# tylerrleee/mcmc-gpu

Measured on AMD Instinct MI355X. Metric: chain-steps/sec on 256x256 grid x 1024 chains; accept-rate parity, higher is better.
Workload: dtype f64; 1 GPU; largeScaleChain 256x256 grid, 1024 chains/GPU, fp64, Philox spectral (Matern 0.9125) proposals, blocks 50-80, sigma_mc 5 (BASELINE configs[1]); chains_total=1024, mh_steps_per_bench_step=2048

## Files before the change

### mcmc_gpu_amd/csrc/chain_strip_kernel.hip

```cpp
#include "gsm_internal.h"
#include "device_util.h"
#include "proposal_device.h"
#include "strip_step.h"
#include <math.h>
#include <stdlib.h>
#include <algorithm>
#include <type_traits>

namespace gsm {

using namespace dev;
using strip::kST;
using strip::kSW;
using strip::kNR;

constexpr int kSUPW = 32 / kSW;
constexpr int kSMAXT = 16 / kSW;

static int strip_tile_len(const BlockTable& B) { return (B.max_bh + 2) * (B.max_bw + 2); }
static int strip_main_len(const FusedArgs& a) { return std::max(a.P.lds_main, strip_tile_len(a.T.B)); }
constexpr int kStripAux = 16 + 32 + 16 + kMathTabDoubles + 4 * kT1S + kMask1D;
size_t fused_strip_lds_doubles(const FusedArgs& a) { return (size_t)strip_main_len(a) + kStripAux; }

bool strip_table_ok(const StaticFields& S, const BlockTable& B, int lds_main, int tiles1_max, int tiles2_max) {
// ... 18 lines not shown
  double* __restrict__ mtab = red2 + 32 + 16;
  double* __restrict__ t1 = mtab + kMathTabDoubles;
  double* __restrict__ m1 = t1 + 4 * kT1S;

  const int tid = threadIdx.x;
  const int lane = tid & 63;
  const int wave = __builtin_amdgcn_readfirstlane(tid >> 6);
  const int chain = blockIdx.x;
  const int n_steps = fa.T.n_steps;
  const int gH = fa.T.S.H, gW = fa.T.S.W;
  const TS* const p_bed = (const TS*)fa.T.beds + (size_t)chain * (size_t)gH * (size_t)gW;
  const TS* const p_en = (const TS*)fa.T.energy + (size_t)chain * (size_t)gH * (size_t)gW;
  const double2* const p_st = fa.T.S.sA;
  const double two_sigma2 = fa.T.S.two_sigma2, rcp_two_sigma2 = fa.T.S.rcp_two_sigma2;
  const uint32_t n_cells = (uint32_t)gH * (uint32_t)gW;
  const crec_t rec0 = (crec_t)(uintptr_t)(fa.P.scalars + (size_t)chain * fa.P.n_steps);
  const uint64_t seed = NOISE ? 0ull : fa.P.seeds[chain];
  for (int i = tid; i < kMathTabDoubles; i += kST) mtab[i] = fa.P.mathtab[i];
  if (tid < 16) red[tid] = 0.0;
  __syncthreads();

  if (tid == 0) {
    const double h0 = fa.T.loss_sum[2 * chain], l0 = fa.T.loss_sum[2 * chain + 1];
    carry[0] = h0; carry[1] = l0; carry[2] = (h0 + l0) / two_sigma2;
  }
  __syncthreads();
  step::Window prev = {};
  const int64_t noise0 = NOISE ? (int64_t)chain * fa.P.n_steps * fa.noise_stride : 0;
  auto prop_rec = [&](crec_t r) {
    PropScalars q;
    q.scale = r->scale; q.nug = r->nug; q.aa = r->aa; q.m_const = r->m_const; q.m_kappa = r->m_kappa;
    q.bh = r->bh; q.bw = r->bw; q.fy_off = r->fy_off; q.g_off = r->g_off; q.pad = r->pad; q.mask_off = r->mask_off;
    q.m_nc = r->m_nc; q.m_m1 = r->m_m1; q.m_bh = r->m_bh; q.m_bw = r->m_bw;
    return q;
  };

  for (int s = 0; s < n_steps; ++s) {
    int ptid = tid;
    asm volatile("" : "+v"(ptid));
    auto relaunder = [&] { asm volatile("" : "+v"(ptid)); };
    const crec_t rec = rec0 + s;
    const int s_row = rec->row, s_col = rec->col, s_bh = rec->bh, s_bw = rec->bw;

    {
      const cargs_t K = kargs();
      const double* __restrict__ g1 = K->P.tab1d;
      if (tid >= kST - kMask1D) m1[tid - (kST - kMask1D)] = K->P.B.mask1d[rec->si * kMask1D + tid - (kST - kMask1D)];
      if (tid < 2 * s_bh) t1[(tid < s_bh) ? tid : kT1S + tid - s_bh] = g1[rec->t1h_off + tid];
      else if (tid >= 256 && tid < 256 + 2 * s_bw) {
        const int i = ptid - 256;
        const double v = g1[rec->t1w_off + i];
        t1[2 * kT1S + ((i < s_bw) ? i : kT1S + i - s_bw)] = (i < s_bw) ? v : -v;
      }
    }
    {
      const cargs_t K = kargs();
      const ProposeArgs pa = load_c(&K->P);
      const PropScalars q = prop_rec(rec);
      const PropGeom pg = prop_geom(pa, q.bh, q.bw);
      NoiseIn nz{nullptr, nullptr, nullptr};
      if (NOISE) {
        const cargs_t F = K;
        const int64_t o = noise0 + (int64_t)s * F->noise_stride;
        nz.re = F->noise_re + o; nz.im = F->noise_im + o;
      }
      coef_items<kST, NOISE, true>(ptid, pa, q, pg, seed, pa.step0 + s, lds, nz, mtab, pa.parseval ? red2 + 16 : nullptr);
    }
    if (step::halo_touches(step::clip_window(gH, gW, s_row, s_col, s_bh, s_bw), prev)) asm volatile("s_waitcnt vmcnt(0)" ::: "memory");
    asm volatile("s_waitcnt lgkmcnt(0)\n\ts_barrier" ::: "memory");
    const double dc0 = lds[0];
    {
      v4f64 uc[kSUPW], us[kSUPW];
      {
        const cargs_t K = kargs();
        const ProposeArgs pa = load_c(&K->P);
        const PropScalars q = prop_rec(rec);
        dft_stage1<kSW, kSUPW, kTabLds1D>(wave, ptid & 63, pa, q, prop_geom(pa, q.bh, q.bw), lds, t1, uc, us);
      }
      asm volatile("s_waitcnt lgkmcnt(0)\n\ts_barrier" ::: "memory");
      {
        const cargs_t K = kargs();
        const ProposeArgs pa = load_c(&K->P);
        relaunder();
        dft_tt_write<kSW, kSUPW>(wave, ptid & 63, prop_geom(pa, s_bh, s_bw), lds, uc, us);
      }
    }
    asm volatile("s_waitcnt lgkmcnt(0)\n\ts_barrier" ::: "memory");
    {
      const cargs_t K = kargs();
      const ProposeArgs pa = load_c(&K->P);
      const PropScalars q = prop_rec(rec);
      const PropGeom pg = prop_geom(pa, q.bh, q.bw);
      const int bw = q.bw;
      v4f64 fe[kSMAXT], fo[kSMAXT];
      const double mreg[kSMAXT][8] = {};
      relaunder();
      const int ln = ptid & 63;
      dft_stage2<kSW, kSMAXT, kTabLds1D>(wave, ln, pa, q, pg, lds, t1 + 2 * kT1S, fe, fo);
      const double gain = standardise<kSW, kSMAXT>(wave, ln, q, pg, dc0, red2, fe, fo, pa.parseval ? red2 + 16 : nullptr);
      NoiseIn nz{nullptr, nullptr, nullptr};
      if (NOISE) {
        const cargs_t F = K;
        const double* nb = F->noise_nug;
        if (nb) nz.nug = nb + noise0 + (int64_t)s * F->noise_stride;
      }
      const bool with_nugget = NOISE ? (nz.nug != nullptr) : (pa.rf.nugget_max > 0.0);
      emit_field<kSW, kSMAXT, kMaskLds1D>(wave, ln, pa, q, pg, fe, fo, mreg, gain, with_nugget, lds, [bw](int y, int x) { return (y + 1) * (bw + 2) + x + 1; }, m1);
      if (with_nugget) {
        __syncthreads();
        relaunder();
        nugget_pass<kST, NOISE>(ptid, pa, q, pg, seed, pa.step0 + s, nz, lds, [bw](int y, int x) { return (y + 1) * (bw + 2) + x + 1; }, mtab);
      }
    }
    relaunder();
    const step::Window Gw = step::clip_window(gH, gW, s_row, s_col, s_bh, s_bw);
    strip::Window G;
    {
      const cargs_t K = kargs();
      G = strip::make_window(gH, gW, s_row, s_col, s_bh, s_bw, K->T.S.tr0, K->T.S.tr1, K->T.S.tc0, K->T.S.tc1);
    }
    const strip::Cfg cfg = strip::config(G.wh, G.ww);
    const strip::Lane L = strip::lane_setup(ptid & 63, wave, cfg, G, gH, gW);
    const rsrc_t r_bed = make_rsrc(p_bed, n_cells * (uint32_t)sizeof(TS));
    const rsrc_t r_en = make_rsrc(p_en, n_cells * (uint32_t)sizeof(TS));
    const rsrc_t r_st = make_rsrc(p_st, 3u * n_cells * 16u);
    uint32_t upd_bits;
    double acc_old;
    bool guard;
    {
      double vb[kNR + 2], ve[kNR];
      double2 a2[strip::kNA];
      if (G.interior) strip::load_state<TS, true>(L, cfg.n, gW, r_bed, r_en, r_st, vb, ve, a2);
      else strip::load_state<TS, false>(L, cfg.n, gW, r_bed, r_en, r_st, vb, ve, a2);
      asm volatile("s_waitcnt lgkmcnt(0)\n\ts_barrier" ::: "memory");
      const int ts = s_bw + 2;
      auto field = [&](int jj, bool) { return lds[L.tidx + jj * ts]; };
      if (G.interior) strip::phase_a<TS, true>(L, cfg.n, gW, s_bw, r_st, field, lds, vb, ve, a2, upd_bits, acc_old, guard);
      else strip::phase_a<TS, false>(L, cfg.n, gW, s_bw, r_st, field, lds, vb, ve, a2, upd_bits, acc_old, guard);
    }
    asm volatile("s_waitcnt lgkmcnt(0)\n\ts_barrier" ::: "memory");
    double en[kNR], vn[kNR];
    {
      double acc_new;
      const cargs_t K = kargs();
      const step::StepConsts SC{K->T.S.res, K->T.S.rcp_res, K->T.S.two_res, K->T.S.rcp_two_res};
      if (G.interior) strip::phase_d<TS, FAST_DIV, true>(L, cfg.n, gW, s_bw, r_st, n_cells * 16u, SC, lds, en, acc_new);
      else strip::phase_d<TS, FAST_DIV, false>(L, cfg.n, gW, s_bw, r_st, n_cells * 16u, SC, lds, en, acc_new);
      double delta = acc_new - acc_old;
      if (guard) delta = INFINITY;
      const double w_delta = wave64_sum(delta);
      if (lane == 0) red[wave] = w_delta;
    }
    strip::read_candidate(L, cfg.n, s_bw, lds, vn);
    const double s_hi = carry[0], s_lo = carry[1];
    double loss_prev = carry[2];
    asm volatile("s_waitcnt lgkmcnt(0)\n\ts_barrier" ::: "memory");
    const double sd = strip::waves_sum(red, lane);
    double c_hi, c_lo, loss_next;
    const bool acc = step::decide<FAST_DIV>(sd, sd == INFINITY, s_hi, s_lo, two_sigma2, rcp_two_sigma2, loss_prev, rec->u, c_hi, c_lo, loss_next);
    if (acc) {
      if (G.interior) strip::commit<TS, true, false>(L, cfg.n, gW, r_bed, r_en, r_en, vn, en, upd_bits);
      else strip::commit<TS, false, false>(L, cfg.n, gW, r_bed, r_en, r_en, vn, en, upd_bits);
      loss_prev = loss_next;
      if (tid == 0) {
        double n_hi, n_lo;
        two_sum(c_hi, c_lo, n_hi, n_lo);
        carry[0] = n_hi; carry[1] = n_lo; carry[2] = loss_next;
      }
      prev = Gw;
    } else {
      prev = step::Window{};
    }
    if (tid == 0) {
      const cargs_t Ke = kargs();
      const StepArgs a = load_c(&Ke->T);
      step::write_record(a, step::record_index(a, chain, s), loss_prev, acc, s_row, s_col, s_bh, s_bw);
    }
  }
  if (tid == 0) {
    fa.T.loss_sum[2 * chain] = carry[0];
    fa.T.loss_sum[2 * chain + 1] = carry[1];
  }
}

template <typename TS, bool FAST_DIV>
__global__ __launch_bounds__(kST, 4) void step_strip_kernel(const StepArgs a) {
  extern __shared__ double tile[];
  __shared__ double red[16];
  __shared__ int tab[2 * 64];
  const StaticFields& S = a.S;
  const int tid = threadIdx.x;
  const int lane = tid & 63;
  const int wave = __builtin_amdgcn_readfirstlane(tid >> 6);
  const int chain = blockIdx.x;
  const int H = S.H, W = S.W;
  const uint32_t n_cells = (uint32_t)H * (uint32_t)W;
  const size_t plane = (size_t)H * W;
  const rsrc_t r_bed = make_rsrc((const TS*)a.beds + (size_t)chain * plane, n_cells * (uint32_t)sizeof(TS));
  const rsrc_t r_en = make_rsrc((const TS*)a.energy + (size_t)chain * plane, n_cells * (uint32_t)sizeof(TS));
  const rsrc_t r_rs = make_rsrc(a.resampled + (size_t)chain * plane, n_cells * 4u);
  const rsrc_t r_st = make_rsrc(S.sA, 3u * n_cells * 16u);
  const step::StepConsts SC{S.res, S.rcp_res, S.two_res, S.rcp_two_res};

// ... 113 lines not shown
```

### mcmc_gpu_amd/csrc/proposal_device.h

```cpp
#pragma once
#include "gsm_internal.h"
#include "device_util.h"
#include "philox.h"
#include "math_tables.h"
#include <math.h>

namespace gsm {

typedef double v4f64 __attribute__((ext_vector_type(4)));

__device__ __forceinline__ uint32_t pmagic(uint32_t d) { return (uint32_t)(0xFFFFFFFFu / d) + 1u; }

__device__ __forceinline__ double fma_sc(double a, double b, double C) {
  double r;
  asm("v_fma_f64 %0, %1, %2, %3" : "=v"(r) : "v"(a), "v"(b), "s"(C));
  return r;
}
__device__ __forceinline__ double mul_sc(double a, double C) {
  double r;
  asm("v_mul_f64 %0, %1, %2" : "=v"(r) : "v"(a), "s"(C));
  return r;
}

__device__ __forceinline__ double exp_lean(double x) {
  const double kf = __builtin_rint(mul_sc(x, 1.44269504088896338700e+00));
  const double r = fma_sc(kf, -1.90821492927058770002e-10, fma_sc(kf, -6.93147180369123816490e-01, x));
  double p = fma_sc(r, 2.08767569878680989792e-09, 2.50521083854417187751e-08);
  p = fma_sc(r, p, 2.75573192239858906526e-07);
  p = fma_sc(r, p, 2.75573192239858906526e-06);
  p = fma_sc(r, p, 2.48015873015873015873e-05);
  p = fma_sc(r, p, 1.98412698412698412698e-04);
  p = fma_sc(r, p, 1.38888888888888888889e-03);
  p = fma_sc(r, p, 8.33333333333333333333e-03);
  p = fma_sc(r, p, 4.16666666666666666667e-02);
  p = fma_sc(r, p, 1.66666666666666666667e-01);
  p = fma_sc(r, p, 0.5);
  p = __fma_rn(r, p, 1.0);
  p = __fma_rn(r, p, 1.0);
  return ldexp(p, (int)kf);
}

__device__ __forceinline__ double sqrt_lean(double t) {
  t = fmax(t, 1e-300);
  const double y = __builtin_amdgcn_rsq(t);
  double g = t * y, h = 0.5 * y;
  const double r = __fma_rn(-h, g, 0.5);
  g = __fma_rn(g, r, g);
  h = __fma_rn(h, r, h);
  return __fma_rn(__fma_rn(-g, g, t), h, g);
}

__device__ __forceinline__ void normals2(uint64_t seed, int64_t step, uint32_t stream, uint32_t idx, double& g1,
                                         double& g2, const double* mt) {
  uint32_t k0 = (uint32_t)(seed & 0xFFFFFFFFu), k1 = (uint32_t)(seed >> 32);
  asm volatile("" : "+s"(k0), "+s"(k1));
  const u32x4 r = philox_draw(((uint64_t)k1 << 32) | k0, step, stream, idx);
  const double u1 = u01_open0_from(r.x, r.y);
  const double u2 = u01_from(r.z, r.w);
  const double rad = sqrt_lean(-2.0 * log_tab(u1, mt));
  double s, c;
  sincos_tab(u2, mt, s, c);
  g1 = rad * c;
  g2 = rad * s;
}

__device__ __forceinline__ void normals4(uint64_t seed, int64_t step, uint32_t stream, uint32_t idx, double& g1, double& g2,
                                         double& h1, double& h2, const double* mt) {
  uint32_t k0 = (uint32_t)(seed & 0xFFFFFFFFu), k1 = (uint32_t)(seed >> 32);
  asm volatile("" : "+s"(k0), "+s"(k1));
  const u32x4 r = philox_draw(((uint64_t)k1 << 32) | k0, step, stream, idx);
  const double ra = sqrt_lean(-2.0 * log_tab(u01_open0_from32(r.x), mt));
  const double rb = sqrt_lean(-2.0 * log_tab(u01_open0_from32(r.z), mt));
  double s, c;
  sincos_tab(u01_from32(r.y), mt, s, c);
  g1 = ra * c; g2 = ra * s;
  sincos_tab(u01_from32(r.w), mt, s, c);
  h1 = rb * c; h2 = rb * s;
}

__device__ __forceinline__ void normals2_key(uint64_t seed, int64_t step, uint32_t stream, uint32_t idx, double& g1, double& g2,
                                             const double* mt) {
  const u32x4 r = philox_draw(seed, step, stream, idx);
  const double u1 = u01_open0_from(r.x, r.y);
  const double u2 = u01_from(r.z, r.w);
  const double rad = sqrt_lean(-2.0 * log_tab(u1, mt));
  double s, c;
  sincos_tab(u2, mt, s, c);
  g1 = rad * c;
  g2 = rad * s;
}

__device__ __forceinline__ double wavenumber(int k, int n, double inv) {
  const int kk = (k < (n + 1) / 2) ? k : k - n;
  return ((double)kk * inv) * 2.0 * M_PI;
}

__device__ __forceinline__ double spectral_amp(const gsm_rf_params& P, const PropScalars& sc, const double k2, const double* mt) {
  if (P.model == GSM_MODEL_GAUSSIAN) return exp_lean(-0.25 * ((sc.aa * sc.aa) * k2));
  if (P.model == GSM_MODEL_EXPONENTIAL) return exp_lean(-0.75 * log_tab(1.0 + (sc.aa * sc.aa) * k2, mt));
  const double nu = (P.smoothness != 0.0) ? P.smoothness : 1.0;
  return exp_lean(__fma_rn(-0.5 * (nu + 1.0), log_tab(sc.m_kappa + 4.0 * M_PI * k2, mt), sc.m_const));
}


struct NoiseIn { const double* re; const double* im; const double* nug; };

__device__ __forceinline__ uint32_t tile_magic(int d) {
  const uint64_t lo = 32769ull | (16385ull << 16) | (10923ull << 32) | (8193ull << 48);
  const uint64_t hi = 6554ull | (5462ull << 16) | (4682ull << 32) | (4097ull << 48);
  if (d > 8) return 32768u / (uint32_t)d + 1u;
  return (uint32_t)(((d <= 4) ? lo : hi) >> (16 * ((d - 1) & 3))) & 0xFFFFu;
}
__device__ __forceinline__ int tile_div(int t, uint32_t magic) { return (int)(((uint32_t)t * magic) >> 15); }

struct PropGeom {
  int bh, bw, hh, hw, ncol, nrow;
  int KR;
  int NR;
  int M1;
  int Kc;
  int N1;
  int SX, ST;
  uint32_t q_mt, q_mt2;
  int hq;
  int NRh;
  int Ke;
  bool split2;
  int hqx, M1h, Kce;
};
__device__ __forceinline__ PropGeom prop_geom(const ProposeArgs& a, int bh, int bw) {
  PropGeom g;
  g.bh = bh; g.bw = bw; g.hh = bh / 2; g.hw = bw / 2;
  g.ncol = g.hw + 1; g.nrow = g.hh + 1;
  g.KR = (g.nrow + 3) & ~3; g.NR = (g.nrow + 15) & ~15;
  g.M1 = (g.ncol + 15) & ~15; g.Kc = (g.ncol + 3) & ~3;
  g.N1 = (bh + 15) & ~15;
  g.SX = a.lds_sx; g.ST = a.lds_st;
  g.q_mt = tile_magic(g.M1 >> 4); g.q_mt2 = tile_magic(g.N1 >> 4);
  g.hq = g.hh >> 1; g.NRh = (g.hq + 16) & ~15; g.Ke = (g.hq + 4) & ~3;
  g.hqx = g.hw >> 1; g.M1h = (g.hqx + 16) & ~15; g.Kce = (g.hqx + 4) & ~3;
  g.split2 = a.split2 && (g.N1 >> 4) * (g.M1h >> 4) <= 8;
  return g;
}

template <int NTH, bool NOISE_IN, bool FOLD_CK = false>
__device__ __forceinline__ void coef_items(const int t, const ProposeArgs& a, const PropScalars& sc, const PropGeom& g,
                                           const uint64_t seed, const int64_t step, double* __restrict__ Pr, const NoiseIn noise,
                                           const double* mt, double* pw_red = nullptr) {
  const gsm_rf_params& P = a.rf;
  const int plane = a.lds_x_half;
  double* __restrict__ Pi = Pr + plane;
  double* __restrict__ Mr = Pi + plane;
  double* __restrict__ Mi = Mr + plane;
  const int SX = g.SX, bh = g.bh, bw = g.bw, hh = g.hh, hw = g.hw, ncol = g.ncol, nrow = g.nrow;
  {
    const int M1 = g.M1, KR = g.KR;
    const uint32_t m_m1 = sc.m_m1;
    for (int i = t; i < (KR - nrow) * M1; i += NTH) {
      const int dy = (int)__umulhi((uint32_t)i, m_m1);
      const int o = (nrow + dy) * SX + (i - dy * M1);
      Pr[o] = 0.0; Pi[o] = 0.0; Mr[o] = 0.0; Mi[o] = 0.0;
    }
    const int kx = ncol + (t & 15);
    if (kx < M1) {
      for (int ky = t >> 4; ky < nrow; ky += NTH / 16) {
        const int o = ky * SX + kx;
        Pr[o] = 0.0; Pi[o] = 0.0; Mr[o] = 0.0; Mi[o] = 0.0;
      }
    }
  }
  const uint32_t m_nc = sc.m_nc;
  double pw = 0.0;
  const double* __restrict__ k2tab = a.k2tab + sc.pad;
  for (int i = t; i < nrow * ncol; i += NTH) {
    const double k2 = k2tab[i];
    const int ky = (int)__umulhi((uint32_t)i, m_nc);
    const int kx = i - ky * ncol;
    const int kyc = bh - ky;
    const bool paired = (ky != 0) && (ky != hh);
    double amp, g1 = 0.0, g2 = 0.0, h1 = 0.0, h2 = 0.0;
    double ar, ai, br = 0.0, bi = 0.0;
    if (NOISE_IN) {
      amp = spectral_amp(P, sc, k2, mt);
      if (FOLD_CK && kx != 0 && kx != hw) amp = 2.0 * amp;
      const int nky = (ky == 0) ? 0 : kyc, nkx = (kx == 0) ? 0 : bw - kx;
      ar = amp * (0.5 * (noise.re[ky * bw + kx] + noise.re[nky * bw + nkx]));
      ai = amp * (0.5 * (noise.im[ky * bw + kx] - noise.im[nky * bw + nkx]));
      if (paired) {
        br = amp * (0.5 * (noise.re[kyc * bw + kx] + noise.re[ky * bw + nkx]));
        bi = amp * (0.5 * (noise.im[kyc * bw + kx] - noise.im[ky * bw + nkx]));
      }
    } else {
      normals4(seed, step, kStreamSpectrum, (uint32_t)(ky * ncol + kx), g1, g2, h1, h2, mt);
      if (!paired) { h1 = 0.0; h2 = 0.0; }
      amp = spectral_amp(P, sc, k2, mt);
      if (FOLD_CK && kx != 0 && kx != hw) amp = 2.0 * amp;
      if (kx > 0 && kx < hw) {
        ar = amp * (g1 * M_SQRT1_2); ai = amp * (g2 * M_SQRT1_2);
        if (paired) { br = amp * (h1 * M_SQRT1_2); bi = amp * (h2 * M_SQRT1_2); }
      } else if (paired) {
        ar = amp * (0.5 * (g1 + h1)); ai = amp * (0.5 * (g2 - h2));
        br = amp * (0.5 * (h1 + g1)); bi = amp * (0.5 * (h2 - g2));
      } else {
        ar = amp * (0.5 * (g1 + g1)); ai = amp * (0.5 * (g2 - g2));
      }
    }
    const int o = ky * SX + kx;
    Pr[o] = ar + br; Pi[o] = ai + bi;
    Mr[o] = paired ? ar - br : 0.0;
    Mi[o] = paired ? ai - bi : 0.0;
    if (pw_red && i != 0) {
      const bool inner = (kx != 0) && (kx != hw);
      const double wc = FOLD_CK ? (inner ? 0.5 : 1.0) : (inner ? 2.0 : 1.0);
      pw += wc * ((ar * ar + ai * ai) + (br * br + bi * bi));
    }
  }
  if (pw_red) {
    const double ws = dev::wave64_sum(pw);
    if ((t & 63) == 0) pw_red[t >> 6] = ws;
  }
}

template <int NW, int AUX = 0>
__device__ __forceinline__ void dma_to_lds(const double* __restrict__ src, double* dst, const int n_doubles, const int w, const int lane) {
  for (int c = w; c < n_doubles / 128; c += NW)
    __builtin_amdgcn_global_load_lds(src + c * 128 + 2 * lane, (__attribute__((address_space(3))) void*)(dst + c * 128), 16, 0, AUX);
}

enum TabMode : int { kTabGlobal2D, kTabLds2D, kTabLds1D };
constexpr int kT1S = 128;
__device__ __forceinline__ uint32_t mod_magic(uint32_t x, uint32_t n, uint32_t magic) { return x - __umulhi(x, magic) * n; }

template <int NW, int UPW, TabMode TABMODE>
__device__ __forceinline__ void dft_stage1(const int w, const int lane, const ProposeArgs& a, const PropScalars& sc, const PropGeom& g,
                                           const double* plds, const double* tabA, v4f64 (&uc)[UPW], v4f64 (&us)[UPW]) {
  const int SX = g.SX, KR = g.KR, NR = g.NR;
  const double* Pr = plds;
  const double* Pi = Pr + a.lds_x_half;
  const double* Mr = Pi + a.lds_x_half;
  const double* Mi = Mr + a.lds_x_half;
  const int l15 = lane & 15, l4 = lane >> 4;
  const int n_mt = g.M1 >> 4;
  const int n_pairs = 2 * n_mt * (g.NRh >> 4);
  const int Ke = g.Ke, bh = g.bh;
  const uint32_t n8 = 8u * (uint32_t)bh;
  const double* __restrict__ T2 = (TABMODE == kTabLds2D) ? tabA : (TABMODE == kTabGlobal2D ? a.tables + sc.fy_off : nullptr);
#pragma unroll
  for (int j = 0; j < UPW; j += 2) {
    const int pq = w + (j >> 1) * NW;
    v4f64 cE = {0.0, 0.0, 0.0, 0.0}, sE = cE, cO = cE, sO = cE;
    if ((j + 1 < UPW) && pq < n_pairs) {
      const int t = pq >> 1;
      const int nt = tile_div(t, g.q_mt), mt = t - nt * n_mt;
      const double* __restrict__ Ac = (pq & 1) ? Pi : Pr;
      const double* __restrict__ As = (pq & 1) ? Mr : Mi;
      const int col = 16 * mt + l15, y = 16 * nt + l15;
      uint32_t mE = 0u, mO = 0u, d8 = 0u;
      if (TABMODE == kTabLds1D) {
        const uint32_t yy = mod_magic((uint32_t)y, (uint32_t)bh, sc.m_bh);
        mE = 8u * mod_magic((uint32_t)(2 * l4) * yy, (uint32_t)bh, sc.m_bh);
        mO = 8u * mod_magic((uint32_t)(2 * l4 + 1) * yy, (uint32_t)bh, sc.m_bh);
        d8 = 8u * mod_magic(8u * yy, (uint32_t)bh, sc.m_bh);
      }
      auto kstep = [&](const int k0, const bool last) {
        int rE = 2 * (k0 + l4), rO = rE + 1;
        const bool vE = rE < KR, vO = rO < KR;
        if (last) { rE = min(rE, KR - 1); rO = min(rO, KR - 1); }
        double aEc = Ac[rE * SX + col], aEs = As[rE * SX + col], aOc = Ac[rO * SX + col], aOs = As[rO * SX + col];
        if (last) {
          if (!vE) { aEc = 0.0; aEs = 0.0; }
          if (!vO) { aOc = 0.0; aOs = 0.0; }
        }
        double bEc, bEs, bOc, bOs;
        if (TABMODE == kTabLds1D) {
          const char* tE = (const char*)tabA + mE;
          const char* tO = (const char*)tabA + mO;
          bEc = *(const double*)tE; bEs = *(const double*)(tE + 8 * kT1S);
          bOc = *(const double*)tO; bOs = *(const double*)(tO + 8 * kT1S);
          mE += d8; mE = min(mE, mE - n8);
          mO += d8; mO = min(mO, mO - n8);
        } else {
          bEc = T2[rE * NR + y]; bEs = T2[KR * NR + rE * NR + y];
          bOc = T2[rO * NR + y]; bOs = T2[KR * NR + rO * NR + y];
        }
        cE = __builtin_amdgcn_mfma_f64_16x16x4f64(aEc, bEc, cE, 0, 0, 0);
        sE = __builtin_amdgcn_mfma_f64_16x16x4f64(aEs, bEs, sE, 0, 0, 0);
        cO = __builtin_amdgcn_mfma_f64_16x16x4f64(aOc, bOc, cO, 0, 0, 0);
        sO = __builtin_amdgcn_mfma_f64_16x16x4f64(aOs, bOs, sO, 0, 0, 0);
      };
      for (int k0 = 0; k0 < Ke - 4; k0 += 4) kstep(k0, false);
      kstep(Ke - 4, true);
    }
    uc[j] = cE; us[j] = sE;
    if (j + 1 < UPW) { uc[j + 1] = cO; us[j + 1] = sO; }
  }
}

template <int NW, int UPW, bool FOLD_CK = false>
__device__ __forceinline__ void dft_tt_write(const int w, const int lane, const PropGeom& g, double* TT, const v4f64 (&uc)[UPW],
                                             const v4f64 (&us)[UPW]) {
  const int l15 = lane & 15, l4 = lane >> 4;
  const int n_mt = g.M1 >> 4;
  const int ST = g.ST, Kc = g.Kc, hh = g.hh, bh = g.bh;
  const int n_pairs = 2 * n_mt * (g.NRh >> 4);
#pragma unroll
  for (int j = 0; j + 1 < UPW; j += 2) {
    const int pq = w + (j >> 1) * NW;
    if (pq < n_pairs) {
      const int t = pq >> 1;
      const bool im = pq & 1;
      const int nt = tile_div(t, g.q_mt), mt = t - nt * n_mt;
      const int y = 16 * nt + l15;
      if (y <= g.hq) {
        const int ym = hh - y;
        double* __restrict__ Th = TT + (im ? Kc * ST : 0);
#pragma unroll
        for (int q = 0; q < 4; ++q) {
          const int kx = 16 * mt + l4 + 4 * q;
          if (kx < Kc) {
            const double U = uc[j][q] + uc[j + 1][q], V = us[j][q] + us[j + 1][q];
            const double Um = uc[j][q] - uc[j + 1][q], Vm = us[j + 1][q] - us[j][q];
            double t1 = im ? U + V : U - V, t2 = im ? U - V : U + V;
            double t3 = im ? Um + Vm : Um - Vm, t4 = im ? Um - Vm : Um + Vm;
            if (FOLD_CK && kx != 0 && kx != g.hw) { t1 = 2.0 * t1; t2 = 2.0 * t2; t3 = 2.0 * t3; t4 = 2.0 * t4; }
            Th[kx * ST + y] = t1;
            if (y > 0 && y < hh) Th[kx * ST + (bh - y)] = t2;
            if (ym != y) {
              Th[kx * ST + ym] = t3;
              if (ym > 0 && ym < hh) Th[kx * ST + (bh - ym)] = t4;
            }
          }
        }
      }
    }
  }
}

struct SlotX { int mt, x; bool ok; };
__device__ __forceinline__ SlotX slot_x(const int w, const int j, const int NW, const int l15, const PropGeom& g) {
  SlotX r;
  const int n_mt2 = g.N1 >> 4;
  if (g.split2) {
    const int tp = w + (j >> 1) * NW;
    const int nt = tile_div(tp, g.q_mt2);
    r.mt = tp - nt * n_mt2;
    const int x0 = 16 * nt + l15;
    r.x = (j & 1) ? g.hw - x0 : x0;
    r.ok = (w >= 0) && tp < n_mt2 * (g.M1h >> 4) && x0 <= g.hqx && !((j & 1) && g.hw - x0 == x0);
  } else {
    const int t = w + j * NW;
    const int nt = tile_div(t, g.q_mt2);
    r.mt = t - nt * n_mt2;
    r.x = 16 * nt + l15;
    r.ok = (w >= 0) && t < n_mt2 * (g.M1 >> 4) && r.x <= g.hw;
  }
  return r;
}

template <int NW, int MAXT, TabMode TABMODE>
__device__ __forceinline__ void dft_stage2(const int w, const int lane, const ProposeArgs& a, const PropScalars& sc, const PropGeom& g,
                                           const double* TT, const double* tabG, v4f64 (&fe)[MAXT], v4f64 (&fo)[MAXT]) {
  const int l15 = lane & 15, l4 = lane >> 4;
  const int ST = g.ST, Kc = g.Kc, M1 = g.M1;
  const int n_mt2 = g.N1 >> 4, n_nt2 = M1 >> 4;
  const int n_t2 = n_mt2 * n_nt2;
  if constexpr (MAXT >= 2) if (g.split2) {
    const int n_tp = n_mt2 * (g.M1h >> 4);
    const int Kce = g.Kce, bw = g.bw;
    const uint32_t n8 = 8u * (uint32_t)bw;
    const double* __restrict__ G2 = (TABMODE == kTabLds2D) ? tabG : (TABMODE == kTabGlobal2D ? a.tables + sc.g_off : nullptr);
#pragma unroll
    for (int j = 0; j + 1 < MAXT; j += 2) {
      const int tp = w + (j >> 1) * NW;
      v4f64 eE = {0.0, 0.0, 0.0, 0.0}, oE = eE, eO = eE, oO = eE;
      if (tp < n_tp) {
        const int nt = tile_div(tp, g.q_mt2), mt = tp - nt * n_mt2;
        const int ycol = 16 * mt + l15, x = 16 * nt + l15;
        uint32_t mE = 0u, mO = 0u, d8 = 0u;
        if (TABMODE == kTabLds1D) {
          const uint32_t xx = mod_magic((uint32_t)x, (uint32_t)bw, sc.m_bw);
          mE = 8u * mod_magic((uint32_t)(2 * l4) * xx, (uint32_t)bw, sc.m_bw);
          mO = 8u * mod_magic((uint32_t)(2 * l4 + 1) * xx, (uint32_t)bw, sc.m_bw);
          d8 = 8u * mod_magic(8u * xx, (uint32_t)bw, sc.m_bw);
        }
        auto kstep = [&](const int k0, const bool last) {
          int rE = 2 * (k0 + l4), rO = rE + 1;
          const bool vE = rE < Kc, vO = rO < Kc;
          if (last) { rE = min(rE, Kc - 1); rO = min(rO, Kc - 1); }
          double aEr = TT[rE * ST + ycol], aEi = TT[(Kc + rE) * ST + ycol], aOr = TT[rO * ST + ycol], aOi = TT[(Kc + rO) * ST + ycol];
          if (last) {
            if (!vE) { aEr = 0.0; aEi = 0.0; }
            if (!vO) { aOr = 0.0; aOi = 0.0; }
          }
          double bEc, bEs, bOc, bOs;
          if (TABMODE == kTabLds1D) {
            const char* tE = (const char*)tabG + mE;
            const char* tO = (const char*)tabG + mO;
            bEc = *(const double*)tE; bEs = *(const double*)(tE + 8 * kT1S);
            bOc = *(const double*)tO; bOs = *(const double*)(tO + 8 * kT1S);
            mE += d8; mE = min(mE, mE - n8);
            mO += d8; mO = min(mO, mO - n8);
          } else {
            bEc = G2[rE * M1 + x]; bEs = G2[Kc * M1 + rE * M1 + x];
            bOc = G2[rO * M1 + x]; bOs = G2[Kc * M1 + rO * M1 + x];
          }
          eE = __builtin_amdgcn_mfma_f64_16x16x4f64(aEr, bEc, eE, 0, 0, 0);
          oE = __builtin_amdgcn_mfma_f64_16x16x4f64(aEi, bEs, oE, 0, 0, 0);
          eO = __builtin_amdgcn_mfma_f64_16x16x4f64(aOr, bOc, eO, 0, 0, 0);
          oO = __builtin_amdgcn_mfma_f64_16x16x4f64(aOi, bOs, oO, 0, 0, 0);
        };
        for (int k0 = 0; k0 < Kce - 4; k0 += 4) kstep(k0, false);
        kstep(Kce - 4, true);
      }
      fe[j] = eE + eO; fo[j] = oE + oO;
      fe[j + 1] = eE - eO; fo[j + 1] = oO - oE;
    }
    return;
  }
  if constexpr (TABMODE == kTabLds1D) {
    struct Tile { const double* a_p; uint32_t m8, d8; bool on; };
    const uint32_t n8 = 8u * (uint32_t)g.bw;
    auto setup = [&](const int j) {
      Tile x{TT, 0u, 0u, false};
      const int t = w + j * NW;
      x.on = (j < MAXT) && (t < n_t2);
      if (x.on) {
        const int nt = tile_div(t, g.q_mt2), mt = t - nt * n_mt2;
        x.a_p = TT + l4 * ST + 16 * mt + l15;
        const uint32_t xx = mod_magic((uint32_t)(16 * nt + l15), (uint32_t)g.bw, sc.m_bw);
        x.m8 = 8u * mod_magic((uint32_t)l4 * xx, (uint32_t)g.bw, sc.m_bw);
        x.d8 = 8u * mod_magic(4u * xx, (uint32_t)g.bw, sc.m_bw);
      }
      return x;
    };
    auto fetch = [&](Tile& x, const int k0, double& a1, double& a2, double& b1, double& b2) {
      const char* tb = (const char*)tabG + x.m8;
      a1 = x.a_p[k0 * ST]; a2 = x.a_p[(Kc + k0) * ST]; b1 = *(const double*)tb; b2 = *(const double*)(tb + 8 * kT1S);
      x.m8 += x.d8;
      x.m8 = min(x.m8, x.m8 - n8);
    };
#pragma unroll
    for (int j = 0; j < MAXT; j += 2) {
      Tile A = setup(j), B = setup(j + 1);
      v4f64 eA = {0.0, 0.0, 0.0, 0.0}, oA = eA, eB = eA, oB = eA;
      if (A.on && B.on) {
        {
          const v4f64 Z = {0.0, 0.0, 0.0, 0.0};
          double a1, a2, b1, b2, a3, a4, b3, b4;
          fetch(A, 0, a1, a2, b1, b2);
          fetch(B, 0, a3, a4, b3, b4);
          eA = __builtin_amdgcn_mfma_f64_16x16x4f64(a1, b1, Z, 0, 0, 0);
          oA = __builtin_amdgcn_mfma_f64_16x16x4f64(a2, b2, Z, 0, 0, 0);
          eB = __builtin_amdgcn_mfma_f64_16x16x4f64(a3, b3, Z, 0, 0, 0);
          oB = __builtin_amdgcn_mfma_f64_16x16x4f64(a4, b4, Z, 0, 0, 0);
        }
        for (int k0 = 4; k0 < Kc; k0 += 4) {
          double a1, a2, b1, b2, a3, a4, b3, b4;
          fetch(A, k0, a1, a2, b1, b2);
          fetch(B, k0, a3, a4, b3, b4);
          eA = __builtin_amdgcn_mfma_f64_16x16x4f64(a1, b1, eA, 0, 0, 0);
          oA = __builtin_amdgcn_mfma_f64_16x16x4f64(a2, b2, oA, 0, 0, 0);
          eB = __builtin_amdgcn_mfma_f64_16x16x4f64(a3, b3, eB, 0, 0, 0);
          oB = __builtin_amdgcn_mfma_f64_16x16x4f64(a4, b4, oB, 0, 0, 0);
        }
      } else if (A.on) {
        int k0 = 0;
        for (; k0 + 8 <= Kc; k0 += 8) {
          double a1, a2, b1, b2, a3, a4, b3, b4;
          fetch(A, k0, a1, a2, b1, b2);
          fetch(A, k0 + 4, a3, a4, b3, b4);
          eA = __builtin_amdgcn_mfma_f64_16x16x4f64(a1, b1, eA, 0, 0, 0);
          oA = __builtin_amdgcn_mfma_f64_16x16x4f64(a2, b2, oA, 0, 0, 0);
          eA = __builtin_amdgcn_mfma_f64_16x16x4f64(a3, b3, eA, 0, 0, 0);
          oA = __builtin_amdgcn_mfma_f64_16x16x4f64(a4, b4, oA, 0, 0, 0);
        }
        if (k0 < Kc) {
          double a1, a2, b1, b2;
          fetch(A, k0, a1, a2, b1, b2);
          eA = __builtin_amdgcn_mfma_f64_16x16x4f64(a1, b1, eA, 0, 0, 0);
          oA = __builtin_amdgcn_mfma_f64_16x16x4f64(a2, b2, oA, 0, 0, 0);
        }
      }
      fe[j] = eA; fo[j] = oA;
      if (j + 1 < MAXT) { fe[j + 1] = eB; fo[j + 1] = oB; }
    }
    return;
  }
  const double* __restrict__ GC = a.tables + sc.g_off;
  const double* __restrict__ GS = GC + Kc * M1;
#pragma unroll
  for (int j = 0; j < MAXT; ++j) {
    v4f64 ae = {0.0, 0.0, 0.0, 0.0}, ao = ae;
    const int t = w + j * NW;
    if (t < n_t2) {
      const int nt = tile_div(t, g.q_mt2), mt = t - nt * n_mt2;
      const double* a_p = TT + l4 * ST + 16 * mt + l15;
      const double* gc_p = GC + l4 * M1 + 16 * nt + l15;
      const double* gs_p = GS + l4 * M1 + 16 * nt + l15;
#pragma unroll 2
      for (int k0 = 0; k0 < Kc; k0 += 4) {
        double gc, gs;
        if (TABMODE == kTabLds2D) {
          const int bo = (l4 + k0) * M1 + 16 * nt + l15;
          gc = tabG[bo]; gs = tabG[Kc * M1 + bo];
        } else {
          gc = gc_p[k0 * M1]; gs = gs_p[k0 * M1];
        }
        ae = __builtin_amdgcn_mfma_f64_16x16x4f64(a_p[k0 * ST], gc, ae, 0, 0, 0);
        ao = __builtin_amdgcn_mfma_f64_16x16x4f64(a_p[(Kc + k0) * ST], gs, ao, 0, 0, 0);
      }
    }
    fe[j] = ae; fo[j] = ao;
  }
}

template <int NW, int MAXT>
__device__ __forceinline__ void mask_prefetch(const int w, const int lane, const ProposeArgs& a, const PropScalars& sc, const PropGeom& g,
                                              double (&mreg)[MAXT][8]) {
  const int l15 = lane & 15, l4 = lane >> 4;
  const int bh = g.bh, bw = g.bw, hw = g.hw;
  const int n_mt2 = g.N1 >> 4, n_t2 = n_mt2 * (g.M1 >> 4);
  const dev::rsrc_t r_mask = dev::make_rsrc(a.B.masks + sc.mask_off, (uint32_t)(bh * bw) * 8u);
#pragma unroll
  for (int j = 0; j < MAXT; ++j) {
    const int t = w + j * NW;
    const int nt = tile_div(t, g.q_mt2), mt = t - nt * n_mt2;
    const int x = 16 * nt + l15;
#pragma unroll
    for (int q = 0; q < 4; ++q) {
      const int y = 16 * mt + l4 + 4 * q;
      const bool ok = (t < n_t2) && (y < bh) && (x <= hw);
      mreg[j][2 * q] = dev::ld_f64<0>(r_mask, ok ? (uint32_t)(y * bw + x) * 8u : dev::kOOB);
      mreg[j][2 * q + 1] = dev::ld_f64<0>(r_mask, (ok && x > 0 && x < hw) ? (uint32_t)(y * bw + bw - x) * 8u : dev::kOOB);
    }
  }
}

template <int NW, int MAXT>
__device__ __forceinline__ double tiles_sum(const double (&part)[MAXT], const int n_tiles, double* red, const int w, const int lane) {
  constexpr int SLOTS = (NW * MAXT > 16) ? 32 : 16;
  static_assert(NW * MAXT >= 16, "every tile slot must have an owner");
  if (w >= 0) {
#pragma unroll
    for (int j = 0; j < MAXT; ++j) {
      const double ws = dev::wave64_sum(part[j]);
      const int t = w + j * NW;
      if (lane == 0 && t < SLOTS) red[t] = (t < n_tiles) ? ws : 0.0;
    }
  }
  asm volatile("s_waitcnt lgkmcnt(0)\n\ts_barrier" ::: "memory");
  double r = dev::row16_sum(red[lane & 15]);
  if (SLOTS == 32) r += dev::row16_sum(red[16 + (lane & 15)]);
  return r;
}

template <int NW, int MAXT>
__device__ __forceinline__ double standardise(const int w, const int lane, const PropScalars& sc, const PropGeom& g, const double dc,
                                              double* red, v4f64 (&fe)[MAXT], v4f64 (&fo)[MAXT], const double* pw_red = nullptr) {
  const int l15 = lane & 15, l4 = lane >> 4;
  const int bh = g.bh, hw = g.hw;
  const int n_mt2 = g.N1 >> 4, n_t2 = n_mt2 * (g.M1 >> 4);
  const int ncell = bh * g.bw;
  const double inv_n = 1.0 / (double)ncell;
  if (pw_red) {
#pragma unroll
    for (int j = 0; j < MAXT; ++j)
#pragma unroll
      for (int q = 0; q < 4; ++q) {
        const double e = fe[j][q], o = fo[j][q];
        fe[j][q] = (e + o) - dc; fo[j][q] = (e - o) - dc;
      }
    asm volatile("s_waitcnt lgkmcnt(0)\n\ts_barrier" ::: "memory");
    double S = pw_red[0];
#pragma unroll
    for (int i = 1; i < NW; ++i) S += pw_red[i];
    const double sd = sqrt(S * inv_n * inv_n);
    return sc.scale / (sd + 1e-12) * inv_n;
  }
  double part[MAXT];
#pragma unroll
  for (int j = 0; j < MAXT; ++j) {
    const SlotX sx = slot_x(w, j, NW, l15, g);
    const int mt = sx.mt, x = sx.x;
    const bool okx = sx.ok;
    const bool twox = okx && (x > 0) && (x < hw);
    double p = 0.0;
#pragma unroll
    for (int q = 0; q < 4; ++q) {
      const int y = 16 * mt + l4 + 4 * q;
      const double e = fe[j][q], o = fo[j][q];
      const double d1 = (e + o) - dc, d2 = (e - o) - dc;
      fe[j][q] = d1; fo[j][q] = d2;
      const double s1 = d1 * d1, s2 = d2 * d2;
      p += (okx && y < bh) ? s1 : 0.0;
      p += (twox && y < bh) ? s2 : 0.0;
    }
    part[j] = p;
  }
  const double sd = sqrt(tiles_sum<NW, MAXT>(part, g.split2 ? 32 : n_t2, red, w, lane) * inv_n * inv_n * inv_n);
  return sc.scale / (sd + 1e-12) * inv_n;
}

enum MaskMode : int { kMaskGlobal, kMaskRegs, kMaskLds1D };
template <int NW, int MAXT, MaskMode MASKMODE, class OMap>
__device__ __forceinline__ void emit_field(const int w, const int lane, const ProposeArgs& a, const PropScalars& sc, const PropGeom& g,
                                           const v4f64 (&fe)[MAXT], const v4f64 (&fo)[MAXT], const double (&mreg)[MAXT][8],
                                           const double gain, const bool with_nugget,
                                           double* __restrict__ out, OMap omap, const double* m1d = nullptr) {
  if (w < 0) return;
  const int l15 = lane & 15, l4 = lane >> 4;
  const int bh = g.bh, bw = g.bw, hw = g.hw;
  const int n_mt2 = g.N1 >> 4, n_t2 = n_mt2 * (g.M1 >> 4);
  const double* __restrict__ mask = a.B.masks + sc.mask_off;
#pragma unroll
  for (int j = 0; j < MAXT; ++j) {
    const SlotX sx = slot_x(w, j, NW, l15, g);
    const int mt = sx.mt, x = sx.x;
#pragma unroll
    for (int q = 0; q < 4; ++q) {
      const int y = 16 * mt + l4 + 4 * q;
      if (sx.ok && (y < bh)) {
#pragma unroll
        for (int half = 0; half < 2; ++half) {
          if (half == 1 && !(x > 0 && x < hw)) continue;
          const int xx = half ? bw - x : x;
          const int o = y * bw + xx;
          const int oi = omap(y, xx);
          const double v = (half ? fo[j][q] : fe[j][q]) * gain;
          double mk;
          if (MASKMODE == kMaskLds1D) mk = m1d[min(min(y, bh - 1 - y), min(xx, bw - 1 - xx))];
          else mk = (MASKMODE == kMaskRegs) ? mreg[j][2 * q + half] : mask[o];
          if (oi >= 0) out[oi] = with_nugget ? v : v * mk;
        }
      }
    }
  }
}

template <int NTH, bool NOISE_IN, class OMap>
__device__ __forceinline__ void nugget_pass(const int t, const ProposeArgs& a, const PropScalars& sc, const PropGeom& g,
                                            const uint64_t seed, const int64_t step, const NoiseIn noise,
                                            double* __restrict__ out, OMap omap, const double* mt) {
  const double* __restrict__ mask = a.B.masks + sc.mask_off;
  const int bw = g.bw, ncell = g.bh * g.bw;
  const double sq_nug = sqrt(sc.nug);
  for (int pr = t; 2 * pr < ncell; pr += NTH) {
    double n1, n2;
    const int o = 2 * pr;
    if (NOISE_IN) { n1 = noise.nug[o]; n2 = noise.nug[o + 1]; }
    else {
      normals2(seed, step, kStreamNugget, (uint32_t)pr, n1, n2, mt);
      n1 *= sq_nug; n2 *= sq_nug;
    }
    const int y = o / bw, x = o - y * bw;
    const int o0 = omap(y, x), o1 = omap(y, x + 1);
    if (o0 >= 0) out[o0] = (out[o0] + n1) * mask[o];
    if (o1 >= 0) out[o1] = (out[o1] + n2) * mask[o + 1];
  }
}

template <int NT, bool NOISE_IN = false, int WIDE = 1, class OMap>
__device__ __forceinline__ void propose_field(const int tid, const ProposeArgs& a, const PropScalars& sc, const uint64_t seed,
                                              const int64_t step, double* plds, double* red, double* __restrict__ out, OMap omap,
                                              const NoiseIn noise = NoiseIn{nullptr, nullptr, nullptr}) {
  constexpr int NW = NT / 64, MAXT = WIDE * 16 / NW, UPW = WIDE * 32 / NW;
  const int lane = tid & 63;
  const int wave = __builtin_amdgcn_readfirstlane(tid >> 6);
  const PropGeom g = prop_geom(a, sc.bh, sc.bw);
  double* mt = red + 32;
  for (int i = tid; i < kMathTabDoubles; i += NT) mt[i] = a.mathtab[i];
  __syncthreads();
  double* pw_red = (a.parseval && NW == 8) ? red + 16 : nullptr;
  coef_items<NT, NOISE_IN>(tid, a, sc, g, seed, step, plds, noise, mt, pw_red);
  __syncthreads();
  const double dc = plds[0];
  v4f64 uc[UPW], us[UPW];
  dft_stage1<NW, UPW, kTabGlobal2D>(wave, lane, a, sc, g, plds, nullptr, uc, us);
  __syncthreads();
  dft_tt_write<NW, UPW>(wave, lane, g, plds, uc, us);
  __syncthreads();
  v4f64 fe[MAXT], fo[MAXT];
  dft_stage2<NW, MAXT, kTabGlobal2D>(wave, lane, a, sc, g, plds, nullptr, fe, fo);
  double mreg[MAXT][8];
  const double gain = standardise<NW, MAXT>(wave, lane, sc, g, dc, red, fe, fo, pw_red);
  const bool with_nugget = NOISE_IN ? (noise.nug != nullptr) : (a.rf.nugget_max > 0.0);
  emit_field<NW, MAXT, kMaskGlobal>(wave, lane, a, sc, g, fe, fo, mreg, gain, with_nugget, out, omap);
  if (with_nugget) {
    __syncthreads();
    nugget_pass<NT, NOISE_IN>(tid, a, sc, g, seed, step, noise, out, omap, mt);
  }
}

}
```

Before: 17.82 million chain-steps/s.

## Pack real/imag DFT columns into shared tiles and skip unneeded stage-2 row tiles

The stage-1 DFT now packs the real and imaginary column halves into one contiguous run of tiles (PACKED mode), so fewer tile pairs are processed. The padding rows of the transpose buffer are zeroed explicitly. When Parseval normalisation is used, the strip window is computed earlier, and stage-2, standardise and emit_field skip output tiles whose rows fall outside the window rows the strip update actually reads. This cuts MFMA, LDS traffic and writes for proposal field rows that are discarded, at the cost of more index arithmetic and a dependency of the proposal on window geometry.

```diff
diff --git a/mcmc_gpu_amd/csrc/chain_strip_kernel.hip b/mcmc_gpu_amd/csrc/chain_strip_kernel.hip
--- a/mcmc_gpu_amd/csrc/chain_strip_kernel.hip
+++ b/mcmc_gpu_amd/csrc/chain_strip_kernel.hip
@@ -124,10 +124,15 @@
         const cargs_t K = kargs();
         const ProposeArgs pa = load_c(&K->P);
         relaunder();
-        dft_tt_write<kSW, kSUPW>(wave, ptid & 63, prop_geom(pa, s_bh, s_bw), lds, uc, us);
-      }
-    }
-    asm volatile("s_waitcnt lgkmcnt(0)\n\ts_barrier" ::: "memory");
+        dft_tt_write<kSW, kSUPW, false, true>(wave, ptid & 63, prop_geom(pa, s_bh, s_bw), lds, uc, us);
+      }
+    }
+    asm volatile("s_waitcnt lgkmcnt(0)\n\ts_barrier" ::: "memory");
+    strip::Window G;
+    {
+      const cargs_t K = kargs();
+      G = strip::make_window(gH, gW, s_row, s_col, s_bh, s_bw, K->T.S.tr0, K->T.S.tr1, K->T.S.tc0, K->T.S.tc1);
+    }
     {
       const cargs_t K = kargs();
       const ProposeArgs pa = load_c(&K->P);
@@ -138,8 +143,10 @@
       const double mreg[kSMAXT][8] = {};
       relaunder();
       const int ln = ptid & 63;
-      dft_stage2<kSW, kSMAXT, kTabLds1D>(wave, ln, pa, q, pg, lds, t1 + 2 * kT1S, fe, fo);
-      const double gain = standardise<kSW, kSMAXT>(wave, ln, q, pg, dc0, red2, fe, fo, pa.parseval ? red2 + 16 : nullptr);
+      RowSpan rs;
+      if (pa.parseval) { rs.y0 = (G.wh > 0) ? G.mr0 : 0; rs.y1 = (G.wh > 0) ? G.mr0 + G.wh : 0; }
+      dft_stage2<kSW, kSMAXT, kTabLds1D>(wave, ln, pa, q, pg, lds, t1 + 2 * kT1S, fe, fo, rs);
+      const double gain = standardise<kSW, kSMAXT>(wave, ln, q, pg, dc0, red2, fe, fo, pa.parseval ? red2 + 16 : nullptr, rs);
       NoiseIn nz{nullptr, nullptr, nullptr};
       if (NOISE) {
         const cargs_t F = K;
@@ -147,7 +154,7 @@
         if (nb) nz.nug = nb + noise0 + (int64_t)s * F->noise_stride;
       }
       const bool with_nugget = NOISE ? (nz.nug != nullptr) : (pa.rf.nugget_max > 0.0);
-      emit_field<kSW, kSMAXT, kMaskLds1D>(wave, ln, pa, q, pg, fe, fo, mreg, gain, with_nugget, lds, [bw](int y, int x) { return (y + 1) * (bw + 2) + x + 1; }, m1);
+      emit_field<kSW, kSMAXT, kMaskLds1D>(wave, ln, pa, q, pg, fe, fo, mreg, gain, with_nugget, lds, [bw](int y, int x) { return (y + 1) * (bw + 2) + x + 1; }, m1, rs);
       if (with_nugget) {
         __syncthreads();
         relaunder();
@@ -156,11 +163,6 @@
     }
     relaunder();
     const step::Window Gw = step::clip_window(gH, gW, s_row, s_col, s_bh, s_bw);
-    strip::Window G;
-    {
-      const cargs_t K = kargs();
-      G = strip::make_window(gH, gW, s_row, s_col, s_bh, s_bw, K->T.S.tr0, K->T.S.tr1, K->T.S.tc0, K->T.S.tc1);
-    }
     const strip::Cfg cfg = strip::config(G.wh, G.ww);
     const strip::Lane L = strip::lane_setup(ptid & 63, wave, cfg, G, gH, gW);
     const rsrc_t r_bed = make_rsrc(p_bed, n_cells * (uint32_t)sizeof(TS));
diff --git a/mcmc_gpu_amd/csrc/proposal_device.h b/mcmc_gpu_amd/csrc/proposal_device.h
--- a/mcmc_gpu_amd/csrc/proposal_device.h
+++ b/mcmc_gpu_amd/csrc/proposal_device.h
@@ -105,11 +105,14 @@
 
 struct NoiseIn { const double* re; const double* im; const double* nug; };
 
-__device__ __forceinline__ uint32_t tile_magic(int d) {
+__device__ __forceinline__ uint32_t tile_magic8(int d) {
   const uint64_t lo = 32769ull | (16385ull << 16) | (10923ull << 32) | (8193ull << 48);
   const uint64_t hi = 6554ull | (5462ull << 16) | (4682ull << 32) | (4097ull << 48);
+  return (uint32_t)(((d <= 4) ? lo : hi) >> (16 * ((d - 1) & 3))) & 0xFFFFu;
+}
+__device__ __forceinline__ uint32_t tile_magic(int d) {
   if (d > 8) return 32768u / (uint32_t)d + 1u;
-  return (uint32_t)(((d <= 4) ? lo : hi) >> (16 * ((d - 1) & 3))) & 0xFFFFu;
+  return tile_magic8(d);
 }
 __device__ __forceinline__ int tile_div(int t, uint32_t magic) { return (int)(((uint32_t)t * magic) >> 15); }
 
@@ -127,6 +130,30 @@
   int Ke;
   bool split2;
   int hqx, M1h, Kce;
+
+  struct PackedRow { int kx; bool im, live; };
+  static __host__ __device__ __forceinline__ PackedRow packed_row(const int c, const int bw) {
+    const int ncol = bw / 2 + 1;
+    PackedRow r;
+    r.live = c < bw;
+    r.im = c >= ncol;
+    r.kx = r.im ? c - ncol + 1 : c;
+    return r;
+  }
+  static __host__ __device__ __forceinline__ int packed_index(const int c, const int bw, const int off_re, const int off_im) {
+    const int ncol = bw / 2 + 1;
+    return c + ((c >= ncol) ? off_im - (ncol - 1) : off_re);
+  }
+  static __host__ __device__ __forceinline__ int packed_tiles(const int bw) { return (bw + 15) >> 4; }
+  static __host__ __device__ __forceinline__ int tt_zero_rows(const int bw) {
+    const int ncol = bw / 2 + 1, Kc = (ncol + 3) & ~3;
+    return 2 + 2 * (Kc - ncol);
+  }
+  static __host__ __device__ __forceinline__ int tt_zero_row(const int r, const int bw) {
+    const int ncol = bw / 2 + 1, Kc = (ncol + 3) & ~3;
+    if (r < 2) return Kc + (r ? bw / 2 : 0);
+    return (((r - 2) & 1) ? Kc : 0) + ncol + ((r - 2) >> 1);
+  }
 };
 __device__ __forceinline__ PropGeom prop_geom(const ProposeArgs& a, int bh, int bw) {
   PropGeom g;
@@ -240,8 +267,10 @@
   const double* Mr = Pi + a.lds_x_half;
   const double* Mi = Mr + a.lds_x_half;
   const int l15 = lane & 15, l4 = lane >> 4;
-  const int n_mt = g.M1 >> 4;
-  const int n_pairs = 2 * n_mt * (g.NRh >> 4);
+  constexpr bool PACKED = TABMODE == kTabLds1D;
+  const int n_mt = PACKED ? PropGeom::packed_tiles(g.bw) : g.M1 >> 4;
+  const uint32_t q_mt = PACKED ? tile_magic8(n_mt) : g.q_mt;
+  const int n_pairs = (PACKED ? 1 : 2) * n_mt * (g.NRh >> 4);
   const int Ke = g.Ke, bh = g.bh;
   const uint32_t n8 = 8u * (uint32_t)bh;
   const double* __restrict__ T2 = (TABMODE == kTabLds2D) ? tabA : (TABMODE == kTabGlobal2D ? a.tables + sc.fy_off : nullptr);
@@ -250,11 +279,12 @@
     const int pq = w + (j >> 1) * NW;
     v4f64 cE = {0.0, 0.0, 0.0, 0.0}, sE = cE, cO = cE, sO = cE;
     if ((j + 1 < UPW) && pq < n_pairs) {
-      const int t = pq >> 1;
-      const int nt = tile_div(t, g.q_mt), mt = t - nt * n_mt;
-      const double* __restrict__ Ac = (pq & 1) ? Pi : Pr;
-      const double* __restrict__ As = (pq & 1) ? Mr : Mi;
-      const int col = 16 * mt + l15, y = 16 * nt + l15;
+      const int t = PACKED ? pq : pq >> 1;
+      const int nt = tile_div(t, q_mt), mt = t - nt * n_mt;
+      const int c = 16 * mt + l15, y = 16 * nt + l15;
+      const double* Ac = PACKED ? Pr + PropGeom::packed_index(c, g.bw, 0, a.lds_x_half) : ((pq & 1) ? Pi : Pr);
+      const double* As = PACKED ? Pr + PropGeom::packed_index(c, g.bw, 3 * a.lds_x_half, 2 * a.lds_x_half) : ((pq & 1) ? Mr : Mi);
+      const int col = PACKED ? 0 : c;
       uint32_t mE = 0u, mO = 0u, d8 = 0u;
       if (TABMODE == kTabLds1D) {
         const uint32_t yy = mod_magic((uint32_t)y, (uint32_t)bh, sc.m_bh);
@@ -296,38 +326,50 @@
   }
 }
 
-template <int NW, int UPW, bool FOLD_CK = false>
+template <int NW, int UPW, bool FOLD_CK = false, bool PACKED = false>
 __device__ __forceinline__ void dft_tt_write(const int w, const int lane, const PropGeom& g, double* TT, const v4f64 (&uc)[UPW],
                                              const v4f64 (&us)[UPW]) {
   const int l15 = lane & 15, l4 = lane >> 4;
-  const int n_mt = g.M1 >> 4;
+  const int n_mt = PACKED ? PropGeom::packed_tiles(g.bw) : g.M1 >> 4;
+  const uint32_t q_mt = PACKED ? tile_magic8(n_mt) : g.q_mt;
   const int ST = g.ST, Kc = g.Kc, hh = g.hh, bh = g.bh;
-  const int n_pairs = 2 * n_mt * (g.NRh >> 4);
+  const int n_pairs = (PACKED ? 1 : 2) * n_mt * (g.NRh >> 4);
+  if (PACKED) {
+    const int nz = PropGeom::tt_zero_rows(g.bw), y = 64 * (w & 1) + lane;
+    for (int r = w >> 1; r < nz; r += NW / 2)
+      if (y < bh) TT[PropGeom::tt_zero_row(r, g.bw) * ST + y] = 0.0;
+  }
 #pragma unroll
   for (int j = 0; j + 1 < UPW; j += 2) {
     const int pq = w + (j >> 1) * NW;
     if (pq < n_pairs) {
-      const int t = pq >> 1;
-      const bool im = pq & 1;
-      const int nt = tile_div(t, g.q_mt), mt = t - nt * n_mt;
+      const int t = PACKED ? pq : pq >> 1;
+      const int nt = tile_div(t, q_mt), mt = t - nt * n_mt;
       const int y = 16 * nt + l15;
       if (y <= g.hq) {
         const int ym = hh - y;
-        double* __restrict__ Th = TT + (im ? Kc * ST : 0);
 #pragma unroll
         for (int q = 0; q < 4; ++q) {
-          const int kx = 16 * mt + l4 + 4 * q;
-          if (kx < Kc) {
+          const int c = 16 * mt + l4 + 4 * q;
+          const bool im = PACKED ? c >= g.ncol : (pq & 1) != 0;
+          double* __restrict__ Th = TT + (PACKED ? PropGeom::packed_index(c, g.bw, 0, Kc) : (im ? Kc : 0) + c) * ST;
+          if (PACKED ? c < g.bw : c < Kc) {
             const double U = uc[j][q] + uc[j + 1][q], V = us[j][q] + us[j + 1][q];
             const double Um = uc[j][q] - uc[j + 1][q], Vm = us[j + 1][q] - us[j][q];
-            double t1 = im ? U + V : U - V, t2 = im ? U - V : U + V;
-            double t3 = im ? Um + Vm : Um - Vm, t4 = im ? Um - Vm : Um + Vm;
-            if (FOLD_CK && kx != 0 && kx != g.hw) { t1 = 2.0 * t1; t2 = 2.0 * t2; t3 = 2.0 * t3; t4 = 2.0 * t4; }
-            Th[kx * ST + y] = t1;
-            if (y > 0 && y < hh) Th[kx * ST + (bh - y)] = t2;
+            const uint64_t flip = im ? 0ull : 1ull << 63;
+            const double sV = __builtin_bit_cast(double, __builtin_bit_cast(uint64_t, V) ^ flip);
+            const double sVm = __builtin_bit_cast(double, __builtin_bit_cast(uint64_t, Vm) ^ flip);
+            double t1 = U + sV, t2 = U - sV;
+            double t3 = Um + sVm, t4 = Um - sVm;
+            if (FOLD_CK) {
+              const int kx = PACKED ? PropGeom::packed_row(c, g.bw).kx : c;
+              if (kx != 0 && kx != g.hw) { t1 = 2.0 * t1; t2 = 2.0 * t2; t3 = 2.0 * t3; t4 = 2.0 * t4; }
+            }
+            Th[y] = t1;
+            if (y > 0 && y < hh) Th[bh - y] = t2;
             if (ym != y) {
-              Th[kx * ST + ym] = t3;
-              if (ym > 0 && ym < hh) Th[kx * ST + (bh - ym)] = t4;
+              Th[ym] = t3;
+              if (ym > 0 && ym < hh) Th[bh - ym] = t4;
             }
           }
         }
@@ -357,9 +399,18 @@
   return r;
 }
 
+struct RowSpan { int y0 = 0, y1 = 1 << 30; };
+__device__ __forceinline__ bool rows_wanted(const int mt, const RowSpan rs) { return 16 * mt < rs.y1 && 16 * mt + 16 > rs.y0; }
+__device__ __forceinline__ bool slot_wanted(const int w, const int j, const int NW, const PropGeom& g, const RowSpan rs) {
+  const int n_mt2 = g.N1 >> 4;
+  const int t = g.split2 ? w + (j >> 1) * NW : w + j * NW;
+  const int nt = tile_div(t, g.q_mt2);
+  return t < n_mt2 * ((g.split2 ? g.M1h : g.M1) >> 4) && rows_wanted(t - nt * n_mt2, rs);
+}
+
 template <int NW, int MAXT, TabMode TABMODE>
 __device__ __forceinline__ void dft_stage2(const int w, const int lane, const ProposeArgs& a, const PropScalars& sc, const PropGeom& g,
-                                           const double* TT, const double* tabG, v4f64 (&fe)[MAXT], v4f64 (&fo)[MAXT]) {
+                                           const double* TT, const double* tabG, v4f64 (&fe)[MAXT], v4f64 (&fo)[MAXT], const RowSpan rs = RowSpan{}) {
   const int l15 = lane & 15, l4 = lane >> 4;
   const int ST = g.ST, Kc = g.Kc, M1 = g.M1;
   const int n_mt2 = g.N1 >> 4, n_nt2 = M1 >> 4;
@@ -373,8 +424,8 @@
     for (int j = 0; j + 1 < MAXT; j += 2) {
       const int tp = w + (j >> 1) * NW;
       v4f64 eE = {0.0, 0.0, 0.0, 0.0}, oE = eE, eO = eE, oO = eE;
-      if (tp < n_tp) {
-        const int nt = tile_div(tp, g.q_mt2), mt = tp - nt * n_mt2;
+      const int nt = tile_div(tp, g.q_mt2), mt = tp - nt * n_mt2;
+      if (tp < n_tp && rows_wanted(mt, rs)) {
         const int ycol = 16 * mt + l15, x = 16 * nt + l15;
         uint32_t mE = 0u, mO = 0u, d8 = 0u;
         if (TABMODE == kTabLds1D) {
@@ -423,9 +474,9 @@
     auto setup = [&](const int j) {
       Tile x{TT, 0u, 0u, false};
       const int t = w + j * NW;
-      x.on = (j < MAXT) && (t < n_t2);
+      const int nt = tile_div(t, g.q_mt2), mt = t - nt * n_mt2;
+      x.on = (j < MAXT) && (t < n_t2) && rows_wanted(mt, rs);
       if (x.on) {
-        const int nt = tile_div(t, g.q_mt2), mt = t - nt * n_mt2;
         x.a_p = TT + l4 * ST + 16 * mt + l15;
         const uint32_t xx = mod_magic((uint32_t)(16 * nt + l15), (uint32_t)g.bw, sc.m_bw);
         x.m8 = 8u * mod_magic((uint32_t)l4 * xx, (uint32_t)g.bw, sc.m_bw);
@@ -463,23 +514,26 @@
           eB = __builtin_amdgcn_mfma_f64_16x16x4f64(a3, b3, eB, 0, 0, 0);
           oB = __builtin_amdgcn_mfma_f64_16x16x4f64(a4, b4, oB, 0, 0, 0);
         }
-      } else if (A.on) {
+      } else if (A.on || B.on) {
+        auto lone = [&](Tile& L, v4f64& eL, v4f64& oL) {
         int k0 = 0;
         for (; k0 + 8 <= Kc; k0 += 8) {
           double a1, a2, b1, b2, a3, a4, b3, b4;
-          fetch(A, k0, a1, a2, b1, b2);
-          fetch(A, k0 + 4, a3, a4, b3, b4);
-          eA = __builtin_amdgcn_mfma_f64_16x16x4f64(a1, b1, eA, 0, 0, 0);
-          oA = __builtin_amdgcn_mfma_f64_16x16x4f64(a2, b2, oA, 0, 0, 0);
-          eA = __builtin_amdgcn_mfma_f64_16x16x4f64(a3, b3, eA, 0, 0, 0);
-          oA = __builtin_amdgcn_mfma_f64_16x16x4f64(a4, b4, oA, 0, 0, 0);
+          fetch(L, k0, a1, a2, b1, b2);
+          fetch(L, k0 + 4, a3, a4, b3, b4);
+          eL = __builtin_amdgcn_mfma_f64_16x16x4f64(a1, b1, eL, 0, 0, 0);
+          oL = __builtin_amdgcn_mfma_f64_16x16x4f64(a2, b2, oL, 0, 0, 0);
+          eL = __builtin_amdgcn_mfma_f64_16x16x4f64(a3, b3, eL, 0, 0, 0);
+          oL = __builtin_amdgcn_mfma_f64_16x16x4f64(a4, b4, oL, 0, 0, 0);
         }
         if (k0 < Kc) {
           double a1, a2, b1, b2;
-          fetch(A, k0, a1, a2, b1, b2);
-          eA = __builtin_amdgcn_mfma_f64_16x16x4f64(a1, b1, eA, 0, 0, 0);
-          oA = __builtin_amdgcn_mfma_f64_16x16x4f64(a2, b2, oA, 0, 0, 0);
-        }
+          fetch(L, k0, a1, a2, b1, b2);
+          eL = __builtin_amdgcn_mfma_f64_16x16x4f64(a1, b1, eL, 0, 0, 0);
+          oL = __builtin_amdgcn_mfma_f64_16x16x4f64(a2, b2, oL, 0, 0, 0);
+        }
+        };
+        if (A.on) lone(A, eA, oA); else lone(B, eB, oB);
       }
       fe[j] = eA; fo[j] = oA;
       if (j + 1 < MAXT) { fe[j + 1] = eB; fo[j + 1] = oB; }
@@ -556,7 +610,8 @@
 
 template <int NW, int MAXT>
 __device__ __forceinline__ double standardise(const int w, const int lane, const PropScalars& sc, const PropGeom& g, const double dc,
-                                              double* red, v4f64 (&fe)[MAXT], v4f64 (&fo)[MAXT], const double* pw_red = nullptr) {
+                                              double* red, v4f64 (&fe)[MAXT], v4f64 (&fo)[MAXT], const double* pw_red = nullptr,
+                                              const RowSpan rs = RowSpan{}) {
   const int l15 = lane & 15, l4 = lane >> 4;
   const int bh = g.bh, hw = g.hw;
   const int n_mt2 = g.N1 >> 4, n_t2 = n_mt2 * (g.M1 >> 4);
@@ -564,12 +619,14 @@
   const double inv_n = 1.0 / (double)ncell;
   if (pw_red) {
 #pragma unroll
-    for (int j = 0; j < MAXT; ++j)
+    for (int j = 0; j < MAXT; ++j) {
+      if (!slot_wanted(w, j, NW, g, rs)) continue;
 #pragma unroll
       for (int q = 0; q < 4; ++q) {
         const double e = fe[j][q], o = fo[j][q];
         fe[j][q] = (e + o) - dc; fo[j][q] = (e - o) - dc;
       }
+    }
     asm volatile("s_waitcnt lgkmcnt(0)\n\ts_barrier" ::: "memory");
     double S = pw_red[0];
 #pragma unroll
@@ -606,7 +663,7 @@
 __device__ __forceinline__ void emit_field(const int w, const int lane, const ProposeArgs& a, const PropScalars& sc, const PropGeom& g,
                                            const v4f64 (&fe)[MAXT], const v4f64 (&fo)[MAXT], const double (&mreg)[MAXT][8],
                                            const double gain, const bool with_nugget,
-                                           double* __restrict__ out, OMap omap, const double* m1d = nullptr) {
+                                           double* __restrict__ out, OMap omap, const double* m1d = nullptr, const RowSpan rs = RowSpan{}) {
   if (w < 0) return;
   const int l15 = lane & 15, l4 = lane >> 4;
   const int bh = g.bh, bw = g.bw, hw = g.hw;
@@ -614,6 +671,7 @@
   const double* __restrict__ mask = a.B.masks + sc.mask_off;
 #pragma unroll
   for (int j = 0; j < MAXT; ++j) {
+    if (!slot_wanted(w, j, NW, g, rs)) continue;
     const SlotX sx = slot_x(w, j, NW, l15, g);
     const int mt = sx.mt, x = sx.x;
 #pragma unroll
```

Measured after the change: 17.78 million chain-steps/s, median of 2. Within noise of the previous version (-0.2%).
